# ConwayBeyond/Funscript-Flow

Hardware: AMD Instinct MI355X
Metric: 1080p frame-pairs/sec (higher is better)
Workload: dtype f32

## Files before the change

### funscript_flow_amd/csrc/ffl_api.hip

```cpp
#include "../../include/ffl.h"
#include "ffl_kernels.h"

#include <math.h>
#include <stdarg.h>
#include <stdio.h>
#include <string.h>

#include <algorithm>
#include <condition_variable>
#include <mutex>
#include <string>
#include <thread>
#include <vector>

#define FFL_EV_RING 16
#define FFL_RAW_RING 4

template <class H, class Arg, hipError_t (*Free)(Arg)>
struct Owned {
    H h = H();
    Owned() = default;
    explicit Owned(H take) : h(take) {}
    Owned(Owned &&o) noexcept : h(o.release()) {}
    Owned &operator=(Owned &&o) noexcept { std::swap(h, o.h); return *this; }
// ... 1119 lines not shown
    return ffl_upload_frames(c, fslot, 1, &data, width, height, channels, stride_bytes);
}

int ffl_download_frame(ffl_ctx *c, int fslot, uint8_t *dst) {
    if (!c) return FFL_ERR_INVALID;
    CtxLock lk(c->mu);
    if (!dst || fslot < 0 || fslot >= c->n_fslots)
        return set_err(c, FFL_ERR_INVALID, "ffl_download_frame: bad frame slot %d", fslot);
    if (!c->frame_valid[fslot]) return set_err(c, FFL_ERR_STATE, "ffl_download_frame: frame slot %d was never uploaded", fslot);
    HIPCHK(c, hipSetDevice(c->device));
    HIPCHK(c, hipMemcpyAsync(dst, c->d_gray + (size_t)fslot * c->N, c->N, hipMemcpyDeviceToHost, c->s_copy));
    HIPCHK(c, hipStreamSynchronize(c->s_copy));
    return FFL_OK;
}

struct DebugCapture {
    int level, iter;
    float *I0, *I1, *R0, *R1, *M, *flow;
};

static int enqueue_batch(ffl_ctx *c, ffl_ctx::Lane &L, const BatchTab &T, int n, int nU, int pov_mode, const DebugCapture *cap) {
    hipStream_t st = L.st;
    const size_t N = c->N;
    const UTab *ut = &L.d_tab->ut;
    const PairTab *pt = &L.d_tab->pt;
    auto pyr_level = [&](int k, hipStream_t s) { ffl_launch_pyr_level(c->d_gray, N, ut, nU, L.pyr[c->geo.levels - k], s); };
    auto expand_level = [&](int k, hipStream_t s) {
        {
            ProfScope ps(c, FFL_K_PYRAMID, s);
            pyr_level(k, s);
        }
        {
            ProfScope ps(c, FFL_K_POLYEXP, s);
            ffl_launch_polyexp(L.poly[c->geo.levels - k], nU, c->pc, s);
        }
    };
    const int mode = cap ? 0 : c->opt.run_ahead;
    if (mode) {
        for (int k = 0; k < (mode == 2 ? 4 : 1); k++)
            if (!L.st_aux[k]) HIPCHK(c, hipStreamCreateWithFlags(L.st_aux[k].put(), hipStreamNonBlocking));
        HIPCHK(c, hipEventRecord(L.ev_fork, st));
        for (int k = c->geo.levels; k >= 0; k--) {
            hipStream_t sa = L.st_aux[mode == 2 ? k : 0];
            if (mode == 2 || k == c->geo.levels) HIPCHK(c, hipStreamWaitEvent(sa, L.ev_fork, 0));
            expand_level(k, sa);
            HIPCHK(c, hipEventRecord(L.ev_R[k], sa));
        }
        if (mode == 2)
            for (int k = c->geo.levels; k >= 0; k--) HIPCHK(c, hipStreamWaitEvent(st, L.ev_R[k], 0));
    }
    const bool run_ahead = mode == 1;
    bool expanded = mode != 0;
    if (mode == 0 && c->opt.merge_expand) {
        {
            ProfScope ps(c, FFL_K_PYRAMID, st);
            if (!ffl_launch_pyr_multi(c->d_gray, N, ut, nU, L.pyr, L.n_jobs, c->opt, st))
                for (int k = c->geo.levels; k >= 0; k--) pyr_level(k, st);
        }
        {
            ProfScope ps(c, FFL_K_POLYEXP, st);
            ffl_launch_polyexp_multi(L.poly, L.n_jobs, nU, c->pc, st);
        }
        expanded = true;
    }

    int pw = 0, ph = 0;
    for (int k = c->geo.levels; k >= 0; k--) {
        const LevelGeom &g = c->geo.lv[k];
        const int lw = g.lw, lh = g.lh;
        const size_t plane = (size_t)lw * lh;
        const size_t I_stride = plane, R_stride = 5 * plane, M_stride = 5 * plane;
        float *Rk = L.d_R + c->lay.r_off[k];
        if (pw == 0 && cap)
            for (int i = 0; i < n; i++) HIPCHK(c, hipMemsetAsync(T.pt.flow[k][i], 0, sizeof(float) * 2 * plane, st));
        if (run_ahead) HIPCHK(c, hipStreamWaitEvent(st, L.ev_R[k], 0));
        else if (!expanded) expand_level(k, st);
        int mi = 0;
        const bool fuse_first = c->opt.fuse_first > 0 && !cap && (long)((lw + 63) / 64) * ((lh + 15) / 16) * n >= c->opt.fuse_first;
        if (!fuse_first) {
            ProfScope ps(c, FFL_K_UPDATE_MATRICES, st);
            ffl_launch_update_matrices(Rk, R_stride, plane, pt, k, n, L.d_M[mi], M_stride, lw, lh, pw, ph, pw == 0, cap != nullptr, c->opt, st);
        }
        bool captured = false;
        auto capture = [&]() -> int {
            HIPCHK(c, hipStreamSynchronize(st));
            if (cap->I0) HIPCHK(c, hipMemcpy(cap->I0, L.d_I + c->lay.i_off[k] + (size_t)T.pt.u0[0] * I_stride, sizeof(float) * plane, hipMemcpyDeviceToHost));
            if (cap->I1) HIPCHK(c, hipMemcpy(cap->I1, L.d_I + c->lay.i_off[k] + (size_t)T.pt.u1[0] * I_stride, sizeof(float) * plane, hipMemcpyDeviceToHost));
            if (cap->R0) HIPCHK(c, hipMemcpy(cap->R0, Rk + (size_t)T.pt.u0[0] * R_stride, sizeof(float) * 5 * plane, hipMemcpyDeviceToHost));
            if (cap->R1) HIPCHK(c, hipMemcpy(cap->R1, Rk + (size_t)T.pt.u1[0] * R_stride, sizeof(float) * 5 * plane, hipMemcpyDeviceToHost));
            if (cap->M) HIPCHK(c, hipMemcpy(cap->M, L.d_M[mi], sizeof(float) * 5 * plane, hipMemcpyDeviceToHost));
            if (cap->flow) HIPCHK(c, hipMemcpy(cap->flow, T.pt.flow[k][0], sizeof(float) * 2 * plane, hipMemcpyDeviceToHost));
            captured = true;
            return FFL_OK;
        };
        for (int it = 0; it < 3; it++) {
            if (cap && cap->level == k && cap->iter == it) {
                int rc = capture();
                if (rc) return rc;
            }
            const int update = it < 2;
            {
                ProfScope ps(c, FFL_K_BLUR_SOLVE, st, it > 0 && !cap);
                if (it == 0 && fuse_first)
                    ffl_launch_blur_solve_first(L.d_M[mi ^ 1], M_stride, Rk, R_stride, plane, pt, k, n, lw, lh, pw, ph, c->opt, st);
                else
                    ffl_launch_blur_solve(L.d_M[mi], L.d_M[mi ^ 1], M_stride, Rk, R_stride, plane, pt, k, n, lw, lh,
                                          update, cap != nullptr, c->opt, st);
            }
            if (update) mi ^= 1;
        }
        if (cap && cap->level == k && !captured) {
            int rc = capture();
            if (rc) return rc;
        }
// ... 1055 lines not shown
```

### funscript_flow_amd/csrc/ffl_kernels.h

```cpp
#pragma once
#include <hip/hip_runtime.h>
#include <limits.h>
#include <stdint.h>

#define FFL_MAXB 256
#define FFL_MAXU (2 * FFL_MAXB)
#define FFL_MAX_LEVELS 4
#define FFL_POLY_N 5
#define FFL_WIN 15
#define FFL_WIN_R 7

struct PolyConsts {
    float g[FFL_POLY_N + 1], xg[FFL_POLY_N + 1], xxg[FFL_POLY_N + 1];
    double gd[FFL_POLY_N + 1], xxgd[FFL_POLY_N + 1];
    double ig11, ig03, ig33, ig55;
};

struct GaussKernel {
    float k[32];
    int ksize;
};

struct UTab {
    int fslot[FFL_MAXU];
// ... 20 lines not shown
enum { FFL_FRONT_GENERIC = 0, FFL_FRONT_AREA2 = 1, FFL_FRONT_IDENTITY = 2 };
enum { FFL_SRC_GRAY = 0, FFL_SRC_BGR = 1, FFL_SRC_YUV = 2, FFL_SRC_YUV16 = 3, FFL_SRC_ANY = -1 };
struct FrameDesc {
    const uint8_t *p0, *p1, *p2;
    long long pitch0, pitch1, pitch2;
    long long ps, cs;
    int c_step;
    int wx, wy;
    int fslot;
};
struct FrontParams {
    int kind, rgb;
    int sw, sh;
    int cx, cy, ow, oh;
    double scale_x, scale_y;
    int mode;
    int shift16, round16;
};
struct ExportTab {
    int slot[FFL_MAXB];
};

enum { FFL_IMP_F32 = 0, FFL_IMP_F16 = 1, FFL_IMP_BF16 = 2 };
enum { FFL_IMP_ANY = 0,
       FFL_IMP_NHWC = 1,
       FFL_IMP_NCHW = 2 };
struct ImportArgs {
    const char *base;
    long long item, pitch, ps, cs;
    float *flow;
    Pass1Result *res;
};

#define FFL_MAX_JOBS 4
enum { FFL_PYR_NONE = -1, FFL_PYR_F1 = 0, FFL_PYR_F2, FFL_PYR_H4, FFL_PYR_H9, FFL_PYR_V4, FFL_PYR_V9, FFL_PYR_H1 };
struct PyrJob {
    int kind, w, h, lw, lh;
    unsigned gx, gy, first, count;
    double sx, sy;
    float *tmp, *I;
    size_t tmp_stride, I_stride;
    GaussKernel gk;
};
struct PyrJobs {
    PyrJob j[FFL_MAX_JOBS];
    int n;
};
struct PolyJob {
    const float *I;
    float *R;
    size_t I_stride, R_stride, plane;
    int w, h;
    unsigned gx, gy, first, count;
};
struct PolyJobs {
    PolyJob j[FFL_MAX_JOBS];
    int n;
};

struct FflOptions {
    int lanes = 2;
    int run_ahead = 0;
    int fuse_first = 10000;
    int merge_expand = 1;
    int use_graph = 1;
    int copy_threads = 4;
    int blur_rows = 0;
    int blur_min_wgs = 3500;
    int tile_order = 0;
    int pyr_coarse = 1;
    int fb_general = 0;
    int import_fused = 1;
};
struct FflOptionRow {
    const char *name;
    int FflOptions::*member;
    int lo, hi;
    bool flag;
};
inline constexpr FflOptionRow kFflOptionRows[] = {
    {"lanes", &FflOptions::lanes, 1, 4, false},
    {"run_ahead", &FflOptions::run_ahead, 0, 2, false},
    {"fuse_first", &FflOptions::fuse_first, 0, INT_MAX, false},
    {"merge_expand", &FflOptions::merge_expand, INT_MIN, INT_MAX, true},
    {"graph", &FflOptions::use_graph, INT_MIN, INT_MAX, true},
    {"copy_threads", &FflOptions::copy_threads, 1, 16, false},
    {"blur_rows", &FflOptions::blur_rows, 0, 64, false},
    {"blur_min_wgs", &FflOptions::blur_min_wgs, 1, INT_MAX, false},
    {"tile_order", &FflOptions::tile_order, 0, 1, false},
    {"pyr_coarse", &FflOptions::pyr_coarse, INT_MIN, INT_MAX, true},
    {"fb_general", &FflOptions::fb_general, 0, 1, false},
    {"import_fused", &FflOptions::import_fused, 0, 1, false},
};

bool ffl_launch_pyr_multi(const uint8_t *gray_base, size_t gray_stride, const UTab *ut, int nU, const PyrJob *levels, int n,
                          const FflOptions &opt, hipStream_t st);
void ffl_launch_polyexp_multi(const PolyJob *levels, int n, int nU, PolyConsts pc, hipStream_t st);
void ffl_launch_frontend(const FrameDesc &d, uint8_t *gray, const FrontParams &p, hipStream_t st);
void ffl_launch_frontend_dev(const FrameDesc *tab, int n, uint8_t *gray_base, size_t N, const FrontParams &p, hipStream_t st);
void ffl_launch_export_flows(const float *flow, const ExportTab &tab, int n, size_t N, char *dst, long long item_stride,
                             int layout, hipStream_t st);
void ffl_launch_import_pass1(const ImportArgs &a, const ExportTab &tab, int n, int dtype, int mode, int w, int h, int pov_mode,
                             int fused, PairTab *pt, unsigned long long *pkey, double *psum, hipStream_t st);
void ffl_launch_gray(const uint8_t *bgr, uint8_t *gray, int n_pixels, hipStream_t st);
size_t ffl_pyr_tmp_floats(int w, int h, int lw);
bool ffl_pyr_level_ok(int w, int h, int lw, int lh, int ksize);
void ffl_launch_pyr_level(const uint8_t *gray_base, size_t gray_stride, const UTab *ut, int nU, const PyrJob &level,
                          hipStream_t st);
void ffl_launch_polyexp(const PolyJob &level, int nU, PolyConsts pc, hipStream_t st);
void ffl_launch_update_matrices(const float *R, size_t R_stride, size_t plane, const PairTab *pt, int level, int nB, float *M,
                                size_t M_stride, int lw, int lh, int pw, int ph, int zero_flow, int store_flow,
                                const FflOptions &opt, hipStream_t st);
void ffl_launch_blur_solve(const float *Min, float *Mout, size_t M_stride, const float *R, size_t R_stride,
                           size_t plane, const PairTab *pt, int level, int nB, int lw, int lh, int update, int store_flow,
                           const FflOptions &opt, hipStream_t st);


void ffl_launch_blur_solve_first(float *Mout, size_t M_stride, const float *R, size_t R_stride, size_t plane,
                                 const PairTab *pt, int level, int nB, int lw, int lh, int pw, int ph, const FflOptions &opt,
                                 hipStream_t st);

#define DIS_MAX_PATCHES 4096
#define DIS_MAX_SCALES 12
struct DisKParams {
    int w, h, finest, coarsest, stride, gd_iters, vr_iters, mean_norm, spatial_prop, stripes;
    float alpha, gamma, delta;
    size_t pair_floats;
    size_t pyr_floats;
    size_t pyr_off[DIS_MAX_SCALES];
    float *dbg;
    int dbg_scale, dbg_stage;
};
void ffl_launch_dis(const UTab *ut, const PairTab *pt, int nB, const uint8_t *gray, size_t gray_stride, float *scratch,
                    const DisKParams &p, hipStream_t st);

int ffl_pass1_blocks(int w, int h);
void ffl_launch_pass1(const PairTab *pt, int nB, int w, int h, int pov_mode, unsigned long long *pkey, double *psum,
                      hipStream_t st);

#define FFL_WINDOW_MAX_RADIUS 32
struct WindowSeq {
    int slot[FFL_MAXB + 2 * FFL_WINDOW_MAX_RADIUS];
};
struct WindowItem {
    const float *flow;
    double cx, cy;
    int cut, pad;
};
struct Pass2Record {
    double dot, cx, cy;
// ... 177 lines not shown
```

### funscript_flow_amd/csrc/kernels_farneback.hip

```cpp
#include "ffl_kernels.h"

__global__ __launch_bounds__(256) void k_gray(const uint8_t *__restrict__ bgr, uint8_t *__restrict__ gray, int n) {
    int i4 = (blockIdx.x * 256 + threadIdx.x) * 4;
    if (i4 + 3 < n) {
        const uint32_t *p = reinterpret_cast<const uint32_t *>(bgr + (size_t)i4 * 3);
        uint32_t a = p[0], b = p[1], c = p[2];
        uint32_t px[12] = {a & 255, (a >> 8) & 255, (a >> 16) & 255, a >> 24, b & 255, (b >> 8) & 255,
                           (b >> 16) & 255, b >> 24, c & 255, (c >> 8) & 255, (c >> 16) & 255, c >> 24};
        uint32_t o = 0;
#pragma unroll
        for (int j = 0; j < 4; j++) {
            uint32_t g = (px[j * 3] * 3735u + px[j * 3 + 1] * 19235u + px[j * 3 + 2] * 9798u + 16384u) >> 15;
            o |= g << (8 * j);
        }
        *reinterpret_cast<uint32_t *>(gray + i4) = o;
    } else {
        for (int i = i4; i < n; i++) {
            uint32_t b = bgr[(size_t)i * 3], g = bgr[(size_t)i * 3 + 1], r = bgr[(size_t)i * 3 + 2];
            gray[i] = (uint8_t)((b * 3735u + g * 19235u + r * 9798u + 16384u) >> 15);
        }
    }
}

void ffl_launch_gray(const uint8_t *bgr, uint8_t *gray, int n_pixels, hipStream_t st) {
    int blocks = (n_pixels + 1023) / 1024;
    hipLaunchKernelGGL(k_gray, dim3(blocks), dim3(256), 0, st, bgr, gray, n_pixels);
}

__device__ __forceinline__ void ffl_resize_coord_half(int d, int src, int &i0, int &i1, float &f) {
    int sx = (d - 1) >> 1;
    float fx = (d & 1) ? 0.25f : 0.75f;
    if (d == 0) { sx = 0; fx = 0.f; }
    if (sx >= src - 1) { sx = src - 1; fx = 0.f; }
    i0 = sx;
    i1 = sx + 1 < src ? sx + 1 : src - 1;
    f = fx;
}

constexpr int ffl_pyr_rows(int R) { return R == 1 ? 16 : (R == 4 ? 8 : 4); }
template <int R>
__device__ __forceinline__ void k_pyr_h2_body(const unsigned bx, const unsigned by, const unsigned bz, const uint8_t *__restrict__ gray_base, size_t gray_stride, const UTab *__restrict__ ut, int w,
                                                int h, int lw, double sx, GaussKernel gk, float *__restrict__ tmp,
                                                size_t tmp_stride) {
    constexpr int ROWS = ffl_pyr_rows(R);
    const int d = bx * 256 + threadIdx.x, u = bz;
    if (d >= lw) return;
    int x0, x1;
    float fx;
    ffl_resize_coord(d, w, sx, x0, x1, fx);
    const bool on1 = fx != 0.f;
    const bool wide = x1 == x0 + 1 && x0 >= R && x1 + R < w && (w & 3) == 0;
    const int wfirst = x0 - R, woff = wfirst & 3, wbase = wfirst - woff;
    int xm[2][R], xp[2][R];
#pragma unroll
    for (int q = 0; q < 2; q++)
#pragma unroll
        for (int t = 1; t <= R; t++) {
            xm[q][t - 1] = ffl_reflect101((q ? x1 : x0) - t, w);
            xp[q][t - 1] = ffl_reflect101((q ? x1 : x0) + t, w);
        }
    const uint8_t *img = gray_base + (size_t)ut->fslot[u] * gray_stride;
    float2 *out = reinterpret_cast<float2 *>(tmp + (size_t)u * tmp_stride) + d;
    const int ybase = by * ROWS;
#pragma unroll
    for (int k = 0; k < ROWS; k++) {
        const int y = min(ybase + k, h - 1);
        const uint8_t *row = img + (size_t)y * w;
        float acc0, acc1 = 0.f;
        if (wide) {
            constexpr int NW = (3 + 2 * R + 2 + 3) / 4;
            const uint32_t *wp = reinterpret_cast<const uint32_t *>(row + wbase);
            uint32_t wd[NW], a[NW];
#pragma unroll
            for (int q2 = 0; q2 < NW; q2++) wd[q2] = wp[q2];
#pragma unroll
            for (int q2 = 0; q2 < NW; q2++)
                a[q2] = q2 + 1 < NW ? __builtin_amdgcn_alignbyte(wd[q2 + 1], wd[q2], woff) : wd[q2] >> (8 * woff);
            auto tap = [&](int j) { return (float)((a[j >> 2] >> (8 * (j & 3))) & 255u); };
            acc0 = gk.k[R] * tap(R);
#pragma unroll
            for (int t = 1; t <= R; t++) acc0 = acc0 + gk.k[R + t] * (tap(R - t) + tap(R + t));
            acc1 = gk.k[R] * tap(R + 1);
#pragma unroll
            for (int t = 1; t <= R; t++) acc1 = acc1 + gk.k[R + t] * (tap(R + 1 - t) + tap(R + 1 + t));
        } else {
            acc0 = gk.k[R] * (float)row[x0];
#pragma unroll
            for (int t = 1; t <= R; t++) acc0 = acc0 + gk.k[R + t] * ((float)row[xm[0][t - 1]] + (float)row[xp[0][t - 1]]);
            if (on1) {
                acc1 = gk.k[R] * (float)row[x1];
#pragma unroll
                for (int t = 1; t <= R; t++)
// ... 62 lines not shown
    }
    if (dyy < lh) I[(size_t)u * I_stride + (size_t)dy * lw + dx] = t[0] * b0 + t[1] * b1;
}
template <int R>
__global__ __launch_bounds__(256) void k_pyr_v2(const float *__restrict__ tmp, size_t tmp_stride, int w, int h, int lw,
                                                int lh, double sx, double sy, GaussKernel gk, float *__restrict__ I,
                                                size_t I_stride) {
    k_pyr_v2_body<R>(blockIdx.x, blockIdx.y, blockIdx.z, tmp, tmp_stride, w, h, lw, lh, sx, sy, gk, I, I_stride);
}

#ifndef FFL_FR1
#define FFL_FR1 8
#define FFL_FR2 2
#endif
template <int S, int FR, bool ALIGNED>
__device__ __forceinline__ void k_pyr_fused3x4_body(const unsigned bx, const unsigned by, const unsigned bz, const uint8_t *__restrict__ gray_base, size_t gray_stride, const UTab *__restrict__ ut,
                                                      int w, int h, int lw, int lh, GaussKernel gk,
                                                      float *__restrict__ I, size_t I_stride) {
    constexpr int NR = S * FR + 2;
    constexpr int NBY = 4 * S + 2;
    const int dx = 4 * (bx * 256 + threadIdx.x), u = bz;
    if (dx >= lw) return;
    const uint8_t *img = gray_base + (size_t)ut->fslot[u] * gray_stride;
    const int cx = S * dx;
    const bool wide = (ALIGNED || (w & 3) == 0) && cx >= 4 && cx + 4 * S + 4 <= w;
    const float k0 = gk.k[1], k1 = gk.k[2];
    const int dy0 = by * FR;
    float H[NR][4 * S];
#pragma unroll
    for (int j = 0; j < NR; j++) {
        const int sy = ffl_reflect101(min(S * dy0 - 1 + j, h + 1), h);
        const uint8_t *row = img + (size_t)sy * w;
        float b[NBY];
        if (wide) {
            uint32_t wd[S + 2];
            if (S == 1) {
                struct __attribute__((packed, aligned(4))) u3 { uint32_t a, b, c; };
                const u3 t = *reinterpret_cast<const u3 *>(row + cx - 4);
                wd[0] = t.a; wd[1] = t.b; wd[2] = t.c;
            } else {
                struct __attribute__((packed, aligned(4))) u4 { uint32_t a, b, c, d; };
                const u4 t = *reinterpret_cast<const u4 *>(row + cx - 4);
                wd[0] = t.a; wd[1] = t.b; wd[2] = t.c; wd[3] = t.d;
            }
            b[0] = (float)(wd[0] >> 24);
#pragma unroll
            for (int t = 0; t < 4 * S; t++) b[1 + t] = (float)((wd[1 + (t >> 2)] >> (8 * (t & 3))) & 255u);
            b[NBY - 1] = (float)(wd[S + 1] & 255u);
        } else {
#pragma unroll
            for (int t = 0; t < NBY; t++) b[t] = (float)row[ffl_reflect101(cx - 1 + t, w)];
        }
#pragma unroll
        for (int c = 0; c < 4 * S; c++) H[j][c] = k0 * b[c + 1] + k1 * (b[c] + b[c + 2]);
    }
#pragma unroll
    for (int o = 0; o < FR; o++) {
        const int dy = dy0 + o;
        if (dy >= lh) break;
        const int c = S * o + 1;
        float out[4];
#pragma unroll
        for (int i = 0; i < 4; i++) {
            if (S == 1) {
                const float v00 = k0 * H[c][i] + k1 * (H[c - 1][i] + H[c + 1][i]);
                out[i] = (v00 * 1.f + 0.f * 0.f) * 1.f + 0.f * 0.f;
            } else {
                const float v00 = k0 * H[c][2 * i] + k1 * (H[c - 1][2 * i] + H[c + 1][2 * i]);
                const float v01 = k0 * H[c][2 * i + 1] + k1 * (H[c - 1][2 * i + 1] + H[c + 1][2 * i + 1]);
                const float v10 = k0 * H[c + 1][2 * i] + k1 * (H[c][2 * i] + H[c + 2][2 * i]);
                const float v11 = k0 * H[c + 1][2 * i + 1] + k1 * (H[c][2 * i + 1] + H[c + 2][2 * i + 1]);
                const float t0 = v00 * 0.5f + v01 * 0.5f, t1 = v10 * 0.5f + v11 * 0.5f;
                out[i] = t0 * 0.5f + t1 * 0.5f;
            }
        }
        float *dst = I + (size_t)u * I_stride + (size_t)dy * lw + dx;
        if (ALIGNED || dx + 3 < lw) {
            ffl_f4u t;
            t.x = out[0]; t.y = out[1]; t.z = out[2]; t.w = out[3];
            *reinterpret_cast<ffl_f4u *>(dst) = t;
        } else {
#pragma unroll
            for (int i = 0; i < 4; i++)
                if (dx + i < lw) dst[i] = out[i];
        }
    }
}
template <int S, int FR, bool ALIGNED>
__global__ __launch_bounds__(256) void k_pyr_fused3x4(const uint8_t *__restrict__ gray_base, size_t gray_stride, const UTab *__restrict__ ut,
                                                      int w, int h, int lw, int lh, GaussKernel gk,
                                                      float *__restrict__ I, size_t I_stride) {
    k_pyr_fused3x4_body<S, FR, ALIGNED>(blockIdx.x, blockIdx.y, blockIdx.z, gray_base, gray_stride, ut, w, h, lw, lh, gk, I, I_stride);
}

#define PC_TW 128
#define PC_TH 64
#define PC_PW 36
#define PC_PH 76
template <int R, int S>
struct PcLevel {
    static constexpr int NC = PC_TW / S;
    static constexpr int NO = NC * (PC_TH / S);
    static constexpr int HROWS = PC_TH + 2 * R - S + 2;
    static constexpr int HROW0 = S / 2 + 5 - R;
    static constexpr int PITCH = 2 * NC + 2;
    static constexpr int B0 = S / 2 + 7 - R;
    static constexpr int ND = (B0 % 4 + 2 * R + 5) / 4;
    static_assert(HROW0 >= 0 && HROW0 + HROWS <= PC_PH && B0 >= 0 && (NC - 1) * (S / 4) + B0 / 4 + ND <= PC_PW, "tile halo");
};
template <int R, int S>
__device__ __forceinline__ void k_pyr_coarse_h(const uint32_t (*sP)[PC_PW], float (*sH)[PcLevel<R, S>::PITCH], const GaussKernel &gk,
                                               int tid) {
    using L = PcLevel<R, S>;
    constexpr int RSTEP = 256 / L::NC, TRIPS = (L::HROWS + RSTEP - 1) / RSTEP, UNROLL = R == 4 ? 3 : TRIPS;
    constexpr int C = L::B0 % 4 + R;
    const int dl = tid % L::NC, rr = tid / L::NC;
#pragma unroll UNROLL
    for (int k = 0; k < TRIPS; k++) {
        const int ry = rr + RSTEP * k;
        if (ry < L::HROWS) {
            const uint32_t *p = &sP[ry + L::HROW0][dl * (S / 4) + L::B0 / 4];
            uint32_t d[L::ND];
#pragma unroll
            for (int q = 0; q < L::ND; q++) d[q] = p[q];
// ... 5 lines not shown
                a1 = a1 + gk.k[R + j] * (tap(C + 1 - j) + tap(C + 1 + j));
            }
            *reinterpret_cast<float2 *>(&sH[ry][2 * dl]) = make_float2(a0, a1);
        }
    }
}
template <int R, int S>
__device__ __forceinline__ void k_pyr_coarse_v(const float (*sH)[PcLevel<R, S>::PITCH], const GaussKernel &gk, int tid, int X0,
                                               int Y0, int w, int h, float *__restrict__ I) {
    using L = PcLevel<R, S>;
    const float a1 = 0.5f, a0 = 1.f - a1, b1 = 0.5f, b0 = 1.f - b1;
    const int lw = w / S, lh = h / S;
#pragma unroll
    for (int k = 0; k < (L::NO + 255) / 256; k++) {
        const int o = tid + 256 * k, el = o / L::NC, dl = o % L::NC;
        if (L::NO % 256 != 0 && o >= L::NO) break;
        const int dx = X0 / S + dl, dy = Y0 / S + el;
        float2 V[2 * R + 2];
#pragma unroll
        for (int j = 0; j < 2 * R + 2; j++) V[j] = *reinterpret_cast<const float2 *>(&sH[S * el + j][2 * dl]);
        float tq[2];
#pragma unroll
        for (int qy = 0; qy < 2; qy++) {
            const int c = R + qy;
            float v0 = gk.k[R] * V[c].x, v1 = gk.k[R] * V[c].y;
#pragma unroll
            for (int j = 1; j <= R; j++) {
                v0 = v0 + gk.k[R + j] * (V[c - j].x + V[c + j].x);
                v1 = v1 + gk.k[R + j] * (V[c - j].y + V[c + j].y);
            }
            tq[qy] = v0 * a0 + v1 * a1;
        }
        if (dx < lw && dy < lh) I[(size_t)dy * lw + dx] = tq[0] * b0 + tq[1] * b1;
    }
}
__global__ __launch_bounds__(256) void k_pyr_coarse(const uint8_t *__restrict__ gray_base, size_t gray_stride,
                                                    const UTab *__restrict__ ut, int w, int h, GaussKernel gk2,
                                                    GaussKernel gk3, float *__restrict__ I2, size_t I2_stride,
                                                    float *__restrict__ I3, size_t I3_stride, int tiles_x, int tiles_y,
                                                    int nU) {
    using L2 = PcLevel<4, 4>;
    using L3 = PcLevel<9, 8>;
    __shared__ __attribute__((aligned(8))) uint32_t sP[PC_PH][PC_PW];
    __shared__ __attribute__((aligned(8))) float sH2[L2::HROWS][L2::PITCH];
    __shared__ __attribute__((aligned(8))) float sH3[L3::HROWS][L3::PITCH];
    const int tid = threadIdx.x;
    const unsigned per = (unsigned)tiles_x * tiles_y;
    unsigned tt;
    if (!ffl_xcd_tile(blockIdx.x, per * nU, tt)) return;
    const int u = tt / per, t = tt - u * per, ty = t / tiles_x, tx = t - ty * tiles_x;
    const int X0 = tx * PC_TW, Y0 = ty * PC_TH;
    const uint8_t *img = gray_base + (size_t)ut->fslot[u] * gray_stride;
    constexpr int PCQ = PC_PW / 4, NLOAD = (PC_PH * PCQ + 255) / 256;
    struct __attribute__((packed, aligned(4))) u4 { uint32_t a, b, c, d; };
#pragma unroll
    for (int k = 0; k < NLOAD; k++) {
        const int i = tid + 256 * k;
        if (i < PC_PH * PCQ) {
            const int ry = i / PCQ, q = i - ry * PCQ;
            const int gy = ffl_reflect101(Y0 - 6 + ry, h), X = X0 - 8 + 16 * q;
            const uint8_t *row = img + (size_t)gy * w;
            uint32_t v[4];
            if (X >= 0 && X + 15 < w) {
                const u4 t4 = *reinterpret_cast<const u4 *>(row + X);
                v[0] = t4.a; v[1] = t4.b; v[2] = t4.c; v[3] = t4.d;
            } else {
#pragma unroll
                for (int c = 0; c < 4; c++) {
                    const int Xc = X + 4 * c;
                    if (Xc >= 0 && Xc + 3 < w)
                        v[c] = *reinterpret_cast<const uint32_t *>(row + Xc);
                    else
                        v[c] = (uint32_t)row[ffl_reflect101(Xc, w)] | ((uint32_t)row[ffl_reflect101(Xc + 1, w)] << 8) |
                               ((uint32_t)row[ffl_reflect101(Xc + 2, w)] << 16) | ((uint32_t)row[ffl_reflect101(Xc + 3, w)] << 24);
                }
            }
            *reinterpret_cast<uint2 *>(&sP[ry][4 * q]) = make_uint2(v[0], v[1]);
            *reinterpret_cast<uint2 *>(&sP[ry][4 * q + 2]) = make_uint2(v[2], v[3]);
        }
    }
    __syncthreads();
    k_pyr_coarse_h<4, 4>(sP, sH2, gk2, tid);
    k_pyr_coarse_h<9, 8>(sP, sH3, gk3, tid);
    __syncthreads();
    k_pyr_coarse_v<4, 4>(sH2, gk2, tid, X0, Y0, w, h, I2 + (size_t)u * I2_stride);
    k_pyr_coarse_v<9, 8>(sH3, gk3, tid, X0, Y0, w, h, I3 + (size_t)u * I3_stride);
}

static bool ffl_pyr_coarse_ok(int w, int h, const PyrJob &l2, const PyrJob &l3) {
    return !((w & 7) || (h & 7) || l2.lw != w / 4 || l2.lh != h / 4 || l3.lw != w / 8 || l3.lh != h / 8 ||
             l2.gk.ksize != 9 || l3.gk.ksize != 19);
}
bool ffl_launch_pyr_coarse(const uint8_t *gray_base, size_t gray_stride, const UTab *ut, int nU, int w, int h,
                           const PyrJob &l2, const PyrJob &l3, hipStream_t st) {
    if (!ffl_pyr_coarse_ok(w, h, l2, l3)) return false;
    const int tiles_x = (w + PC_TW - 1) / PC_TW, tiles_y = (h + PC_TH - 1) / PC_TH;
    hipLaunchKernelGGL(k_pyr_coarse, dim3(ffl_xcd_blocks((unsigned)tiles_x * tiles_y * nU)), dim3(256), 0, st, gray_base,
                       gray_stride, ut, w, h, l2.gk, l3.gk, l2.I, l2.I_stride, l3.I, l3.I_stride, tiles_x, tiles_y, nU);
    return true;
}

__global__ __launch_bounds__(256) void k_pyr_multi(const uint8_t *__restrict__ gray_base, size_t gray_stride, const UTab *__restrict__ ut,
                                                   PyrJobs jobs) {
    int i = 0;
#pragma unroll
    for (int t = 1; t < FFL_MAX_JOBS; t++)
        if (t < jobs.n && blockIdx.x >= jobs.j[t].first) i = t;
    const PyrJob &J = jobs.j[i];
    unsigned t;
    if (!ffl_xcd_tile(blockIdx.x - J.first, J.count, t)) return;
    const unsigned per = J.gx * J.gy;
    const unsigned bz = t / per, r = t - bz * per, by = r / J.gx, bx = r - by * J.gx;
    switch (J.kind) {
        case FFL_PYR_F1: k_pyr_fused3x4_body<1, FFL_FR1, true>(bx, by, bz, gray_base, gray_stride, ut, J.w, J.h, J.lw, J.lh, J.gk, J.I, J.I_stride); break;
        case FFL_PYR_F2: k_pyr_fused3x4_body<2, FFL_FR2, true>(bx, by, bz, gray_base, gray_stride, ut, J.w, J.h, J.lw, J.lh, J.gk, J.I, J.I_stride); break;
        case FFL_PYR_H4: k_pyr_h2_body<4>(bx, by, bz, gray_base, gray_stride, ut, J.w, J.h, J.lw, J.sx, J.gk, J.tmp, J.tmp_stride); break;
        case FFL_PYR_H9: k_pyr_h2_body<9>(bx, by, bz, gray_base, gray_stride, ut, J.w, J.h, J.lw, J.sx, J.gk, J.tmp, J.tmp_stride); break;
        case FFL_PYR_V4: k_pyr_v2_body<4>(bx, by, bz, J.tmp, J.tmp_stride, J.w, J.h, J.lw, J.lh, J.sx, J.sy, J.gk, J.I, J.I_stride); break;
        default: k_pyr_v2_body<9>(bx, by, bz, J.tmp, J.tmp_stride, J.w, J.h, J.lw, J.lh, J.sx, J.sy, J.gk, J.I, J.I_stride); break;
    }
}

struct PyrForm {
    int kind;
    bool aligned;
    bool merged;
    unsigned gx, gy;
    unsigned vx, vy;
};
// ... 56 lines not shown
            V.gy = f.vy;
            V.first = tb;
            V.count = V.gx * V.gy * (unsigned)nU;
            tb += ffl_xcd_blocks(V.count);
            B.j[B.n++] = V;
        }
        J.first = ta;
        J.count = J.gx * J.gy * (unsigned)nU;
        ta += ffl_xcd_blocks(J.count);
        A.j[A.n++] = J;
    }
    if (A.n) hipLaunchKernelGGL(k_pyr_multi, dim3(ta), dim3(256), 0, st, gray_base, gray_stride, ut, A);
    if (B.n) hipLaunchKernelGGL(k_pyr_multi, dim3(tb), dim3(256), 0, st, gray_base, gray_stride, ut, B);
    return true;
}

template <int S, int FR>
static void ffl_launch_pyr_fused(const uint8_t *gray_base, size_t gray_stride, const UTab *ut, int nU, const PyrJob &J,
                                 const PyrForm &f, hipStream_t st) {
    const auto kern = f.aligned ? &k_pyr_fused3x4<S, FR, true> : &k_pyr_fused3x4<S, FR, false>;
    hipLaunchKernelGGL(kern, dim3(f.gx, f.gy, nU), dim3(256), 0, st, gray_base, gray_stride, ut, J.w, J.h, J.lw, J.lh, J.gk, J.I,
                       J.I_stride);
}
template <int R>
static void ffl_launch_pyr_hv(const uint8_t *gray_base, size_t gray_stride, const UTab *ut, int nU, const PyrJob &J,
                              const PyrForm &f, hipStream_t st) {
    hipLaunchKernelGGL(k_pyr_h2<R>, dim3(f.gx, f.gy, nU), dim3(256), 0, st, gray_base, gray_stride, ut, J.w, J.h, J.lw, J.sx,
                       J.gk, J.tmp, J.tmp_stride);
    hipLaunchKernelGGL(k_pyr_v2<R>, dim3(f.vx, f.vy, nU), dim3(256), 0, st, J.tmp, J.tmp_stride, J.w, J.h, J.lw, J.lh, J.sx,
                       J.sy, J.gk, J.I, J.I_stride);
}
void ffl_launch_pyr_level(const uint8_t *gray_base, size_t gray_stride, const UTab *ut, int nU, const PyrJob &J,
                          hipStream_t st) {
    const PyrForm f = ffl_pyr_form(J.w, J.h, J.lw, J.lh, J.gk.ksize);
    switch (f.kind) {
        case FFL_PYR_F1: ffl_launch_pyr_fused<1, FFL_FR1>(gray_base, gray_stride, ut, nU, J, f, st); break;
        case FFL_PYR_F2: ffl_launch_pyr_fused<2, FFL_FR2>(gray_base, gray_stride, ut, nU, J, f, st); break;
        case FFL_PYR_H1: ffl_launch_pyr_hv<1>(gray_base, gray_stride, ut, nU, J, f, st); break;
        case FFL_PYR_H4: ffl_launch_pyr_hv<4>(gray_base, gray_stride, ut, nU, J, f, st); break;
        case FFL_PYR_H9: ffl_launch_pyr_hv<9>(gray_base, gray_stride, ut, nU, J, f, st); break;
        default: break;
    }
}

#ifndef PE_TW
#define PE_TW 64
#define PE_TH 16
#endif
#define PE_N FFL_POLY_N
#define PE_LW (PE_TW + 2 * PE_N)
#define PE_LQ ((PE_LW + 3) / 4)
#define PE_PITCH (4 * PE_LQ)

__device__ __forceinline__ void k_polyexp_body(const unsigned bx, const unsigned by, const unsigned bz, const float *__restrict__ I, size_t I_stride, float *__restrict__ R,
                                                 size_t R_stride, size_t plane, int w, int h, PolyConsts pc) {
    __shared__ __attribute__((aligned(16))) float sI[PE_TH + 2 * PE_N][PE_PITCH];
    __shared__ __attribute__((aligned(16))) float sV[3][PE_TH][PE_PITCH];
    const int tid = threadIdx.x;
    const int u = bz;
    const int x0 = bx * PE_TW, y0 = by * PE_TH;
    const float *img = I + (size_t)u * I_stride;

    constexpr int N_IN = (PE_TH + 2 * PE_N) * PE_LQ, N_V = PE_TH * PE_LQ;
#pragma unroll
    for (int it = 0; it < (N_IN + 255) / 256; it++) {
        const int i = tid + 256 * it;
        if (i < N_IN) {
            const int ly = i / PE_LQ, lx = 4 * (i - ly * PE_LQ);
            const int gy = min(max(y0 + ly - PE_N, 0), h - 1), gx = x0 + lx - PE_N;
            const float *row = img + (size_t)gy * w;
            float4 t;
            if (gx >= 0 && gx + 3 < w) {
                const ffl_f4u q = *reinterpret_cast<const ffl_f4u *>(row + gx);
                t = make_float4(q.x, q.y, q.z, q.w);
            } else {
                t = make_float4(row[min(max(gx, 0), w - 1)], row[min(max(gx + 1, 0), w - 1)],
                                row[min(max(gx + 2, 0), w - 1)], row[min(max(gx + 3, 0), w - 1)]);
            }
            *reinterpret_cast<float4 *>(&sI[ly][lx]) = t;
        }
    }
    __syncthreads();

#pragma unroll
    for (int it = 0; it < (N_V + 255) / 256; it++) {
        const int i = tid + 256 * it;
        if (i >= N_V) break;
        const int ly = i / PE_LQ, lx = 4 * (i - ly * PE_LQ);
        const float4 c4 = *reinterpret_cast<const float4 *>(&sI[ly + PE_N][lx]);
        const float c[4] = {c4.x, c4.y, c4.z, c4.w};
        float r0[4], r1[4], r2[4];
#pragma unroll
        for (int e = 0; e < 4; e++) {
            r0[e] = c[e] * pc.g[0];
            r1[e] = 0.f;
            r2[e] = 0.f;
        }
#pragma unroll
        for (int k = 1; k <= PE_N; k++) {
            const float4 a4 = *reinterpret_cast<const float4 *>(&sI[ly + PE_N - k][lx]);
            const float4 b4 = *reinterpret_cast<const float4 *>(&sI[ly + PE_N + k][lx]);
            const float a[4] = {a4.x, a4.y, a4.z, a4.w}, b[4] = {b4.x, b4.y, b4.z, b4.w};
#pragma unroll
            for (int e = 0; e < 4; e++) {
                const float p = a[e] + b[e], d = b[e] - a[e];
                r0[e] = r0[e] + pc.g[k] * p;
                r1[e] = r1[e] + pc.xg[k] * d;
                r2[e] = r2[e] + pc.xxg[k] * p;
            }
        }
        *reinterpret_cast<float4 *>(&sV[0][ly][lx]) = make_float4(r0[0], r0[1], r0[2], r0[3]);
        *reinterpret_cast<float4 *>(&sV[1][ly][lx]) = make_float4(r1[0], r1[1], r1[2], r1[3]);
        *reinterpret_cast<float4 *>(&sV[2][ly][lx]) = make_float4(r2[0], r2[1], r2[2], r2[3]);
    }
    __syncthreads();

    float *out = R + (size_t)u * R_stride;
    {
        static_assert(PE_TW * PE_TH == 1024 && PE_TW % 4 == 0, "one 4-pixel item per lane");
        const int ly = tid / (PE_TW / 4), lx = 4 * (tid % (PE_TW / 4));
        const int x = x0 + lx, y = y0 + ly;
        if (x >= w || y >= h) return;
        float t[3][16];
#pragma unroll
        for (int p = 0; p < 3; p++) {
            const float *src = &sV[p][ly][lx];
#pragma unroll
            for (int q = 0; q < 3; q++) {
                const float4 v = *reinterpret_cast<const float4 *>(src + 4 * q);
                t[p][4 * q] = v.x; t[p][4 * q + 1] = v.y; t[p][4 * q + 2] = v.z; t[p][4 * q + 3] = v.w;
            }
            const float2 v2 = *reinterpret_cast<const float2 *>(src + 12);
            t[p][12] = v2.x; t[p][13] = v2.y;
        }
        float o[5][4];
        const float g0c = pc.g[0];
#pragma unroll
        for (int e = 0; e < 4; e++) {
            const int c = PE_N + e;
            double b1 = (double)(t[0][c] * g0c), b2 = 0, b3 = (double)(t[1][c] * g0c), b4 = 0, b5 = (double)(t[2][c] * g0c), b6 = 0;
#pragma unroll
            for (int k = 1; k <= PE_N; k++) {
                const float gk = pc.g[k], xgk = pc.xg[k];
                const float s0 = t[0][c + k] + t[0][c - k];
                const float d0 = (t[0][c + k] - t[0][c - k]) * xgk;
                const float s1 = (t[1][c + k] + t[1][c - k]) * gk;
                const float d1 = (t[1][c + k] - t[1][c - k]) * xgk;
                const float s2 = (t[2][c + k] + t[2][c - k]) * gk;
                const double tg = (double)s0;
                b1 = __builtin_fma(tg, pc.gd[k], b1);
                b4 = __builtin_fma(tg, pc.xxgd[k], b4);
                b2 += (double)d0;
                b3 += (double)s1;
                b6 += (double)d1;
                b5 += (double)s2;
            }
            o[0][e] = (float)(b3 * pc.ig11);
            o[1][e] = (float)(b2 * pc.ig11);
            o[2][e] = (float)(b1 * pc.ig03 + b5 * pc.ig33);
            o[3][e] = (float)(b1 * pc.ig03 + b4 * pc.ig33);
            o[4][e] = (float)(b6 * pc.ig55);
        }
        const size_t off = (size_t)y * w + x;
        if (x + 3 < w) {
#pragma unroll
            for (int c = 0; c < 5; c++) {
                ffl_f4u q;
                q.x = o[c][0]; q.y = o[c][1]; q.z = o[c][2]; q.w = o[c][3];
                *reinterpret_cast<ffl_f4u *>(out + c * plane + off) = q;
            }
        } else {
#pragma unroll
            for (int c = 0; c < 5; c++)
#pragma unroll
                for (int e = 0; e < 4; e++)
                    if (x + e < w) out[c * plane + off + e] = o[c][e];
        }
    }
}
__global__ __launch_bounds__(256) void k_polyexp(const float *__restrict__ I, size_t I_stride, float *__restrict__ R,
                                                 size_t R_stride, size_t plane, int w, int h, PolyConsts pc) {
    k_polyexp_body(blockIdx.x, blockIdx.y, blockIdx.z, I, I_stride, R, R_stride, plane, w, h, pc);
}

__global__ __launch_bounds__(256) void k_polyexp_multi(PolyJobs jobs, PolyConsts pc) {
    int i = 0;
#pragma unroll
    for (int t = 1; t < FFL_MAX_JOBS; t++)
        if (t < jobs.n && blockIdx.x >= jobs.j[t].first) i = t;
    const PolyJob &J = jobs.j[i];
    const unsigned t = blockIdx.x - J.first;
    if (t >= J.count) return;
    const unsigned per = J.gx * J.gy;
    const unsigned bz = t / per, r = t - bz * per, by = r / J.gx, bx = r - by * J.gx;
    k_polyexp_body(bx, by, bz, J.I, J.I_stride, J.R, J.R_stride, J.plane, J.w, J.h, pc);
}

void ffl_launch_polyexp_multi(const PolyJob *jobs_in, int n, int nU, PolyConsts pc, hipStream_t st) {
    PolyJobs jobs = {};
    unsigned total = 0;
    for (int i = 0; i < n; i++) {
        jobs.j[i] = jobs_in[i];
        jobs.j[i].gx = (jobs_in[i].w + PE_TW - 1) / PE_TW;
        jobs.j[i].gy = (jobs_in[i].h + PE_TH - 1) / PE_TH;
        jobs.j[i].first = total;
        jobs.j[i].count = jobs.j[i].gx * jobs.j[i].gy * (unsigned)nU;
        total += jobs.j[i].count;
    }
    jobs.n = n;
    hipLaunchKernelGGL(k_polyexp_multi, dim3(total), dim3(256), 0, st, jobs, pc);
}

void ffl_launch_polyexp(const PolyJob &J, int nU, PolyConsts pc, hipStream_t st) {
    dim3 grid((J.w + PE_TW - 1) / PE_TW, (J.h + PE_TH - 1) / PE_TH, nU);
    hipLaunchKernelGGL(k_polyexp, grid, dim3(256), 0, st, J.I, J.I_stride, J.R, J.R_stride, J.plane, J.w, J.h, pc);
}

__device__ __forceinline__ float2 ffl_upsample2(const float4 c0, const float4 c1, bool first0, bool first1, float a1, float b1) {
    const float a0 = 1.f - a1, b0 = 1.f - b1;
    const float2 p00 = first0 ? make_float2(c0.x, c0.y) : make_float2(c0.z, c0.w);
    const float2 p01 = first1 ? make_float2(c0.x, c0.y) : make_float2(c0.z, c0.w);
    const float2 p10 = first0 ? make_float2(c1.x, c1.y) : make_float2(c1.z, c1.w);
    const float2 p11 = first1 ? make_float2(c1.x, c1.y) : make_float2(c1.z, c1.w);
    float2 f;
    float t0 = p00.x * a0 + p01.x * a1, t1 = p10.x * a0 + p11.x * a1;
    f.x = (t0 * b0 + t1 * b1) * 2.0f;
    t0 = p00.y * a0 + p01.y * a1;
    t1 = p10.y * a0 + p11.y * a1;
    f.y = (t0 * b0 + t1 * b1) * 2.0f;
    return f;
}

template <int NR, typename Disp, typename Keep>
__device__ __forceinline__ void ffl_um_rows(const float *R0, const float *R1, float *M, size_t plane, int w, int h, int x,
                                            bool xin, int ybase, Disp disp, Keep keep) {
    struct UmRow {
        float2 f;
        float a00, a01, a10, a11;
        bool inside;
        float r0[5];
        ffl_f2u t[5], u[5];
    };
    auto issue = [&](int k) {
        UmRow S;
        const int y = min(ybase + 4 * k, h - 1);
        S.f = disp(k);
        const unsigned o = (unsigned)y * (unsigned)w + (unsigned)x;
#pragma unroll
        for (int c = 0; c < 5; c++) S.r0[c] = *ffl_at<float>(R0 + c * plane, o);
        const UmLoc L = ffl_um_locate(w, h, x, y, S.f.x, S.f.y);
        S.a00 = L.a00; S.a01 = L.a01; S.a10 = L.a10; S.a11 = L.a11; S.inside = L.inside;
        const unsigned o1 = L.inside ? (unsigned)L.y1 * (unsigned)w + (unsigned)L.x1 : 0u;
#pragma unroll
        for (int c = 0; c < 5; c++) {
            S.t[c] = ffl_ld_corner(R1 + c * plane, o1);
            S.u[c] = ffl_ld_corner(R1 + c * plane, o1 + (unsigned)w);
        }
        return S;
    };
    UmRow cur = issue(0);
#pragma unroll
    for (int k = 0; k < NR; k++) {
        UmRow nxt;
// ... 467 lines not shown
```

Measured before the change: 6272.

## Fuse level-0 pyramid blur into polynomial expansion reading gray u8 directly

When the finest pyramid level is a plain 3-tap blur (F1 form), the polyexp kernel now loads the u8 gray tile itself, applies the separable 3-tap blur in shared memory, and feeds the result to the polynomial expansion. The pyramid launch skips that level when no capture is requested. This removes a full-resolution float write and re-read of the level-0 image per frame. The cost is extra shared-memory work and sync points inside polyexp, plus a second boundary-handling path.

Result: faster. 6357, median of 6 (+1.4%).

```diff
diff --git a/funscript_flow_amd/csrc/ffl_api.hip b/funscript_flow_amd/csrc/ffl_api.hip
--- a/funscript_flow_amd/csrc/ffl_api.hip
+++ b/funscript_flow_amd/csrc/ffl_api.hip
@@ -1195,14 +1195,17 @@
     const bool run_ahead = mode == 1;
     bool expanded = mode != 0;
     if (mode == 0 && c->opt.merge_expand) {
+        const PyrJob *l0 = &L.pyr[L.n_jobs - 1];
+        const bool fuse_l0 = c->opt.fuse_l0_blur && ffl_polyexp_from_gray_ok(*l0);
+        const int skip_l0 = fuse_l0 && !cap;
         {
             ProfScope ps(c, FFL_K_PYRAMID, st);
-            if (!ffl_launch_pyr_multi(c->d_gray, N, ut, nU, L.pyr, L.n_jobs, c->opt, st))
-                for (int k = c->geo.levels; k >= 0; k--) pyr_level(k, st);
+            if (!ffl_launch_pyr_multi(c->d_gray, N, ut, nU, L.pyr, L.n_jobs - skip_l0, c->opt, st))
+                for (int k = c->geo.levels; k >= skip_l0; k--) pyr_level(k, st);
         }
         {
             ProfScope ps(c, FFL_K_POLYEXP, st);
-            ffl_launch_polyexp_multi(L.poly, L.n_jobs, nU, c->pc, st);
+            ffl_launch_polyexp_multi(L.poly, L.n_jobs, nU, c->pc, c->d_gray, N, ut, fuse_l0 ? l0 : nullptr, st);
         }
         expanded = true;
     }
diff --git a/funscript_flow_amd/csrc/ffl_kernels.h b/funscript_flow_amd/csrc/ffl_kernels.h
--- a/funscript_flow_amd/csrc/ffl_kernels.h
+++ b/funscript_flow_amd/csrc/ffl_kernels.h
@@ -96,6 +96,8 @@
     size_t I_stride, R_stride, plane;
     int w, h;
     unsigned gx, gy, first, count;
+    int from_gray;
+    float gk0, gk1;
 };
 struct PolyJobs {
     PolyJob j[FFL_MAX_JOBS];
@@ -113,6 +115,7 @@
     int blur_min_wgs = 3500;
     int tile_order = 0;
     int pyr_coarse = 1;
+    int fuse_l0_blur = 1;
     int fb_general = 0;
     int import_fused = 1;
 };
@@ -133,13 +136,16 @@
     {"blur_min_wgs", &FflOptions::blur_min_wgs, 1, INT_MAX, false},
     {"tile_order", &FflOptions::tile_order, 0, 1, false},
     {"pyr_coarse", &FflOptions::pyr_coarse, INT_MIN, INT_MAX, true},
+    {"fuse_l0_blur", &FflOptions::fuse_l0_blur, INT_MIN, INT_MAX, true},
     {"fb_general", &FflOptions::fb_general, 0, 1, false},
     {"import_fused", &FflOptions::import_fused, 0, 1, false},
 };
 
 bool ffl_launch_pyr_multi(const uint8_t *gray_base, size_t gray_stride, const UTab *ut, int nU, const PyrJob *levels, int n,
                           const FflOptions &opt, hipStream_t st);
-void ffl_launch_polyexp_multi(const PolyJob *levels, int n, int nU, PolyConsts pc, hipStream_t st);
+bool ffl_polyexp_from_gray_ok(const PyrJob &l0);
+void ffl_launch_polyexp_multi(const PolyJob *levels, int n, int nU, PolyConsts pc, const uint8_t *gray_base, size_t gray_stride,
+                              const UTab *ut, const PyrJob *l0, hipStream_t st);
 void ffl_launch_frontend(const FrameDesc &d, uint8_t *gray, const FrontParams &p, hipStream_t st);
 void ffl_launch_frontend_dev(const FrameDesc *tab, int n, uint8_t *gray_base, size_t N, const FrontParams &p, hipStream_t st);
 void ffl_launch_export_flows(const float *flow, const ExportTab &tab, int n, size_t N, char *dst, long long item_stride,
diff --git a/funscript_flow_amd/csrc/kernels_farneback.hip b/funscript_flow_amd/csrc/kernels_farneback.hip
--- a/funscript_flow_amd/csrc/kernels_farneback.hip
+++ b/funscript_flow_amd/csrc/kernels_farneback.hip
@@ -38,6 +38,27 @@
 }
 
 constexpr int ffl_pyr_rows(int R) { return R == 1 ? 16 : (R == 4 ? 8 : 4); }
+
+__device__ __forceinline__ float ffl_blur3(float m, float c, float p, float k0, float k1) { return k0 * c + k1 * (m + p); }
+__device__ __forceinline__ float ffl_lerp_identity(float v) { return (v * 1.f + 0.f * 0.f) * 1.f + 0.f * 0.f; }
+
+__device__ __forceinline__ void ffl_gray16_reflect101(const uint8_t *__restrict__ row, int X, int w, bool words, uint32_t (&v)[4]) {
+    struct __attribute__((packed, aligned(4))) u4 { uint32_t a, b, c, d; };
+    if (words && X >= 0 && X + 15 < w) {
+        const u4 t4 = *reinterpret_cast<const u4 *>(row + X);
+        v[0] = t4.a; v[1] = t4.b; v[2] = t4.c; v[3] = t4.d;
+    } else {
+#pragma unroll
+        for (int c = 0; c < 4; c++) {
+            const int Xc = X + 4 * c;
+            if (words && Xc >= 0 && Xc + 3 < w)
+                v[c] = *reinterpret_cast<const uint32_t *>(row + Xc);
+            else
+                v[c] = (uint32_t)row[ffl_reflect101(Xc, w)] | ((uint32_t)row[ffl_reflect101(Xc + 1, w)] << 8) |
+                       ((uint32_t)row[ffl_reflect101(Xc + 2, w)] << 16) | ((uint32_t)row[ffl_reflect101(Xc + 3, w)] << 24);
+        }
+    }
+}
 template <int R>
 __device__ __forceinline__ void k_pyr_h2_body(const unsigned bx, const unsigned by, const unsigned bz, const uint8_t *__restrict__ gray_base, size_t gray_stride, const UTab *__restrict__ ut, int w,
                                                 int h, int lw, double sx, GaussKernel gk, float *__restrict__ tmp,
@@ -206,7 +227,7 @@
             for (int t = 0; t < NBY; t++) b[t] = (float)row[ffl_reflect101(cx - 1 + t, w)];
         }
 #pragma unroll
-        for (int c = 0; c < 4 * S; c++) H[j][c] = k0 * b[c + 1] + k1 * (b[c] + b[c + 2]);
+        for (int c = 0; c < 4 * S; c++) H[j][c] = ffl_blur3(b[c], b[c + 1], b[c + 2], k0, k1);
     }
 #pragma unroll
     for (int o = 0; o < FR; o++) {
@@ -217,13 +238,12 @@
 #pragma unroll
         for (int i = 0; i < 4; i++) {
             if (S == 1) {
-                const float v00 = k0 * H[c][i] + k1 * (H[c - 1][i] + H[c + 1][i]);
-                out[i] = (v00 * 1.f + 0.f * 0.f) * 1.f + 0.f * 0.f;
+                out[i] = ffl_lerp_identity(ffl_blur3(H[c - 1][i], H[c][i], H[c + 1][i], k0, k1));
             } else {
-                const float v00 = k0 * H[c][2 * i] + k1 * (H[c - 1][2 * i] + H[c + 1][2 * i]);
-                const float v01 = k0 * H[c][2 * i + 1] + k1 * (H[c - 1][2 * i + 1] + H[c + 1][2 * i + 1]);
-                const float v10 = k0 * H[c + 1][2 * i] + k1 * (H[c][2 * i] + H[c + 2][2 * i]);
-                const float v11 = k0 * H[c + 1][2 * i + 1] + k1 * (H[c][2 * i + 1] + H[c + 2][2 * i + 1]);
+                const float v00 = ffl_blur3(H[c - 1][2 * i], H[c][2 * i], H[c + 1][2 * i], k0, k1);
+                const float v01 = ffl_blur3(H[c - 1][2 * i + 1], H[c][2 * i + 1], H[c + 1][2 * i + 1], k0, k1);
+                const float v10 = ffl_blur3(H[c][2 * i], H[c + 1][2 * i], H[c + 2][2 * i], k0, k1);
+                const float v11 = ffl_blur3(H[c][2 * i + 1], H[c + 1][2 * i + 1], H[c + 2][2 * i + 1], k0, k1);
                 const float t0 = v00 * 0.5f + v01 * 0.5f, t1 = v10 * 0.5f + v11 * 0.5f;
                 out[i] = t0 * 0.5f + t1 * 0.5f;
             }
@@ -335,7 +355,6 @@
     const int X0 = tx * PC_TW, Y0 = ty * PC_TH;
     const uint8_t *img = gray_base + (size_t)ut->fslot[u] * gray_stride;
     constexpr int PCQ = PC_PW / 4, NLOAD = (PC_PH * PCQ + 255) / 256;
-    struct __attribute__((packed, aligned(4))) u4 { uint32_t a, b, c, d; };
 #pragma unroll
     for (int k = 0; k < NLOAD; k++) {
         const int i = tid + 256 * k;
@@ -344,20 +363,7 @@
             const int gy = ffl_reflect101(Y0 - 6 + ry, h), X = X0 - 8 + 16 * q;
             const uint8_t *row = img + (size_t)gy * w;
             uint32_t v[4];
-            if (X >= 0 && X + 15 < w) {
-                const u4 t4 = *reinterpret_cast<const u4 *>(row + X);
-                v[0] = t4.a; v[1] = t4.b; v[2] = t4.c; v[3] = t4.d;
-            } else {
-#pragma unroll
-                for (int c = 0; c < 4; c++) {
-                    const int Xc = X + 4 * c;
-                    if (Xc >= 0 && Xc + 3 < w)
-                        v[c] = *reinterpret_cast<const uint32_t *>(row + Xc);
-                    else
-                        v[c] = (uint32_t)row[ffl_reflect101(Xc, w)] | ((uint32_t)row[ffl_reflect101(Xc + 1, w)] << 8) |
-                               ((uint32_t)row[ffl_reflect101(Xc + 2, w)] << 16) | ((uint32_t)row[ffl_reflect101(Xc + 3, w)] << 24);
-                }
-            }
+            ffl_gray16_reflect101(row, X, w, true, v);
             *reinterpret_cast<uint2 *>(&sP[ry][4 * q]) = make_uint2(v[0], v[1]);
             *reinterpret_cast<uint2 *>(&sP[ry][4 * q + 2]) = make_uint2(v[2], v[3]);
         }
@@ -520,8 +526,11 @@
 #define PE_LQ ((PE_LW + 3) / 4)
 #define PE_PITCH (4 * PE_LQ)
 
+#define PE_UH (PE_TH + 2 * PE_N + 2)
+#define PE_UW (PE_LQ + 1)
 __device__ __forceinline__ void k_polyexp_body(const unsigned bx, const unsigned by, const unsigned bz, const float *__restrict__ I, size_t I_stride, float *__restrict__ R,
-                                                 size_t R_stride, size_t plane, int w, int h, PolyConsts pc) {
+                                                 size_t R_stride, size_t plane, int w, int h, PolyConsts pc,
+                                                 const uint8_t *__restrict__ gimg = nullptr, float gk0 = 0.f, float gk1 = 0.f) {
     __shared__ __attribute__((aligned(16))) float sI[PE_TH + 2 * PE_N][PE_PITCH];
     __shared__ __attribute__((aligned(16))) float sV[3][PE_TH][PE_PITCH];
     const int tid = threadIdx.x;
@@ -530,22 +539,77 @@
     const float *img = I + (size_t)u * I_stride;
 
     constexpr int N_IN = (PE_TH + 2 * PE_N) * PE_LQ, N_V = PE_TH * PE_LQ;
-#pragma unroll
-    for (int it = 0; it < (N_IN + 255) / 256; it++) {
-        const int i = tid + 256 * it;
-        if (i < N_IN) {
-            const int ly = i / PE_LQ, lx = 4 * (i - ly * PE_LQ);
-            const int gy = min(max(y0 + ly - PE_N, 0), h - 1), gx = x0 + lx - PE_N;
-            const float *row = img + (size_t)gy * w;
-            float4 t;
-            if (gx >= 0 && gx + 3 < w) {
-                const ffl_f4u q = *reinterpret_cast<const ffl_f4u *>(row + gx);
-                t = make_float4(q.x, q.y, q.z, q.w);
-            } else {
-                t = make_float4(row[min(max(gx, 0), w - 1)], row[min(max(gx + 1, 0), w - 1)],
-                                row[min(max(gx + 2, 0), w - 1)], row[min(max(gx + 3, 0), w - 1)]);
-            }
-            *reinterpret_cast<float4 *>(&sI[ly][lx]) = t;
+    if (gimg) {
+        static_assert(PE_TW % 8 == 0 && PE_UW % 4 == 0 && 4 * PE_UW >= PE_PITCH + 4, "u8 tile: 16-byte pieces from x0 - 8 on");
+        static_assert(sizeof(uint32_t) * PE_UH * PE_UW <= sizeof(sV[0]) && sizeof(float) * PE_UH * PE_PITCH <= 2 * sizeof(sV[0]),
+                      "the u8 tile and its horizontal blur fit the dead sV");
+        uint32_t (*sU)[PE_UW] = reinterpret_cast<uint32_t (*)[PE_UW]>(&sV[0][0][0]);
+        float (*sH)[PE_PITCH] = reinterpret_cast<float (*)[PE_PITCH]>(&sV[1][0][0]);
+        const bool words = (w & 3) == 0;
+        if (tid < PE_UH * (PE_UW / 4)) {
+            const int r = tid / (PE_UW / 4), q = tid - r * (PE_UW / 4);
+            uint32_t v[4];
+            ffl_gray16_reflect101(gimg + (size_t)ffl_reflect101(y0 - PE_N - 1 + r, h) * w, x0 - 8 + 16 * q, w, words, v);
+            *reinterpret_cast<uint4 *>(&sU[r][4 * q]) = make_uint4(v[0], v[1], v[2], v[3]);
+        }
+        __syncthreads();
+        constexpr int N_H = PE_UH * PE_LQ;
+#pragma unroll
+        for (int it = 0; it < (N_H + 255) / 256; it++) {
+            const int i = tid + 256 * it;
+            if (i < N_H) {
+                const int r = i / PE_LQ, lx = 4 * (i - r * PE_LQ), gx = x0 + lx - PE_N;
+                float b[4];
+                if (gx >= 0 && gx + 3 < w) {
+                    const uint32_t d0 = sU[r][lx / 4], d1 = sU[r][lx / 4 + 1];
+                    const float t[6] = {(float)((d0 >> 16) & 255u), (float)(d0 >> 24), (float)(d1 & 255u),
+                                        (float)((d1 >> 8) & 255u), (float)((d1 >> 16) & 255u), (float)(d1 >> 24)};
+#pragma unroll
+                    for (int e = 0; e < 4; e++) b[e] = ffl_blur3(t[e], t[e + 1], t[e + 2], gk0, gk1);
+                } else {
+                    const uint8_t *ub = reinterpret_cast<const uint8_t *>(sU[r]);
+#pragma unroll
+                    for (int e = 0; e < 4; e++) {
+                        const int c = min(max(gx + e, 0), w - 1) - (x0 - 8);
+                        b[e] = ffl_blur3((float)ub[c - 1], (float)ub[c], (float)ub[c + 1], gk0, gk1);
+                    }
+                }
+                *reinterpret_cast<float4 *>(&sH[r][lx]) = make_float4(b[0], b[1], b[2], b[3]);
+            }
+        }
+        __syncthreads();
+#pragma unroll
+        for (int it = 0; it < (N_IN + 255) / 256; it++) {
+            const int i = tid + 256 * it;
+            if (i < N_IN) {
+                const int ly = i / PE_LQ, lx = 4 * (i - ly * PE_LQ);
+                const int r = min(max(y0 + ly - PE_N, 0), h - 1) - (y0 - PE_N - 1);
+                const float4 m = *reinterpret_cast<const float4 *>(&sH[r - 1][lx]);
+                const float4 c = *reinterpret_cast<const float4 *>(&sH[r][lx]);
+                const float4 p = *reinterpret_cast<const float4 *>(&sH[r + 1][lx]);
+                *reinterpret_cast<float4 *>(&sI[ly][lx]) =
+                    make_float4(ffl_lerp_identity(ffl_blur3(m.x, c.x, p.x, gk0, gk1)), ffl_lerp_identity(ffl_blur3(m.y, c.y, p.y, gk0, gk1)),
+                                ffl_lerp_identity(ffl_blur3(m.z, c.z, p.z, gk0, gk1)), ffl_lerp_identity(ffl_blur3(m.w, c.w, p.w, gk0, gk1)));
+            }
+        }
+    } else {
+#pragma unroll
+        for (int it = 0; it < (N_IN + 255) / 256; it++) {
+            const int i = tid + 256 * it;
+            if (i < N_IN) {
+                const int ly = i / PE_LQ, lx = 4 * (i - ly * PE_LQ);
+                const int gy = min(max(y0 + ly - PE_N, 0), h - 1), gx = x0 + lx - PE_N;
+                const float *row = img + (size_t)gy * w;
+                float4 t;
+                if (gx >= 0 && gx + 3 < w) {
+                    const ffl_f4u q = *reinterpret_cast<const ffl_f4u *>(row + gx);
+                    t = make_float4(q.x, q.y, q.z, q.w);
+                } else {
+                    t = make_float4(row[min(max(gx, 0), w - 1)], row[min(max(gx + 1, 0), w - 1)],
+                                    row[min(max(gx + 2, 0), w - 1)], row[min(max(gx + 3, 0), w - 1)]);
+                }
+                *reinterpret_cast<float4 *>(&sI[ly][lx]) = t;
+            }
         }
     }
     __syncthreads();
@@ -651,7 +715,8 @@
     k_polyexp_body(blockIdx.x, blockIdx.y, blockIdx.z, I, I_stride, R, R_stride, plane, w, h, pc);
 }
 
-__global__ __launch_bounds__(256) void k_polyexp_multi(PolyJobs jobs, PolyConsts pc) {
+__global__ __launch_bounds__(256) void k_polyexp_multi(PolyJobs jobs, PolyConsts pc, const uint8_t *__restrict__ gray_base,
+                                                       size_t gray_stride, const UTab *__restrict__ ut) {
     int i = 0;
 #pragma unroll
     for (int t = 1; t < FFL_MAX_JOBS; t++)
@@ -661,10 +726,14 @@
     if (t >= J.count) return;
     const unsigned per = J.gx * J.gy;
     const unsigned bz = t / per, r = t - bz * per, by = r / J.gx, bx = r - by * J.gx;
-    k_polyexp_body(bx, by, bz, J.I, J.I_stride, J.R, J.R_stride, J.plane, J.w, J.h, pc);
-}
-
-void ffl_launch_polyexp_multi(const PolyJob *jobs_in, int n, int nU, PolyConsts pc, hipStream_t st) {
+    const uint8_t *gimg = J.from_gray ? gray_base + (size_t)ut->fslot[bz] * gray_stride : nullptr;
+    k_polyexp_body(bx, by, bz, J.I, J.I_stride, J.R, J.R_stride, J.plane, J.w, J.h, pc, gimg, J.gk0, J.gk1);
+}
+
+bool ffl_polyexp_from_gray_ok(const PyrJob &l0) { return ffl_pyr_form(l0.w, l0.h, l0.lw, l0.lh, l0.gk.ksize).kind == FFL_PYR_F1; }
+
+void ffl_launch_polyexp_multi(const PolyJob *jobs_in, int n, int nU, PolyConsts pc, const uint8_t *gray_base, size_t gray_stride,
+                              const UTab *ut, const PyrJob *l0, hipStream_t st) {
     PolyJobs jobs = {};
     unsigned total = 0;
     for (int i = 0; i < n; i++) {
@@ -676,7 +745,12 @@
         total += jobs.j[i].count;
     }
     jobs.n = n;
-    hipLaunchKernelGGL(k_polyexp_multi, dim3(total), dim3(256), 0, st, jobs, pc);
+    if (l0) {
+        jobs.j[n - 1].from_gray = 1;
+        jobs.j[n - 1].gk0 = l0->gk.k[1];
+        jobs.j[n - 1].gk1 = l0->gk.k[2];
+    }
+    hipLaunchKernelGGL(k_polyexp_multi, dim3(total), dim3(256), 0, st, jobs, pc, gray_base, gray_stride, ut);
 }
 
 void ffl_launch_polyexp(const PolyJob &J, int nU, PolyConsts pc, hipStream_t st) {
```
